# czi-ai/scldm

Hardware: AMD Instinct MI355X
Metric: cells/sec (whole node) @100 Euler steps; DiT-fwd MFMA util % of peak (higher is better)
Workload: dtype bf16; 1 GPU; dentate_b4096_euler100; cells_per_gpu=4096, global_cells=4096, cfg_evaluations=100, method=euler, sample_forwards_per_evaluation_per_gpu=12288, gathered_rows=8192, parallelism=single GPU

## Files before the change

scldm_amd/csrc/api.hip:

```cpp
#include <hip/hip_runtime.h>

#include <algorithm>
#include <cstdarg>
#include <cstdio>
#include <cstdlib>
#include <cstring>
#include <vector>

#include <cmath>
#include "api_common.hpp"
#include "dit_aux.hpp"
#include "dit_forward.hpp"
#include "dit_handle.hpp"
#include "ode_rk.hpp"

using namespace scldm;

static thread_local char g_err[512] = "";
int scldm_fail(int code, const char* fmt, ...) {
  va_list ap;
  va_start(ap, fmt);
  vsnprintf(g_err, sizeof(g_err), fmt, ap);
  va_end(ap);
  return code;
// ... 28 lines not shown
    if (cfg->n_embed % 256 != 0 || cfg->n_embed > 2048 || cfg->seq_len != 16 || (hd != 32 && hd != 64))
      return fail(SCLDM_ERR_SHAPE, "unsupported DiT shape: fused kernels need n_embed=256, n_head=8, seq_len=16; the generic path needs "
                  "n_embed %% 256 == 0 (<= 2048), seq_len=16, head_dim 32 or 64 (got n_embed=%d, n_head=%d, seq_len=%d)", cfg->n_embed,
                  cfg->n_head, cfg->seq_len);
  }
  if (cfg->n_layer < 1 || cfg->hidden_dim < 1) return fail(SCLDM_ERR_SHAPE, "bad n_layer / hidden_dim");
  if (cfg->n_classes < 0 || cfg->n_classes > SCLDM_MAX_CLASSES) return fail(SCLDM_ERR_SHAPE, "n_classes must be <= %d", SCLDM_MAX_CLASSES);
  if (cfg->has_null_row != 0 && cfg->has_null_row != 1) return fail(SCLDM_ERR_SHAPE, "has_null_row must be 0 or 1");
  for (int c = 0; c < cfg->n_classes; ++c)
    if (cfg->class_vocab[c] < 1) return fail(SCLDM_ERR_SHAPE, "class %d has an empty vocabulary", c);
  scldm_dit* h = new scldm_dit();
  h->cfg = *cfg;
  h->fused = fused;
  h->mod_w = cfg->n_layer * 6 * cfg->n_embed + 2 * cfg->n_embed;
  for (int c = 0; c < cfg->n_classes; ++c) h->tab_rows[c] = cfg->class_vocab[c] + cfg->has_null_row;
  h->bf16_sources = true;
  if (const char* e = getenv("SCLDM_TRAIN_BF16_SOURCES")) h->bf16_sources = atoi(e) != 0;
  h->wgrad_batch = true;
  if (const char* e = getenv("SCLDM_WGRAD_BATCH")) h->wgrad_batch = atoi(e) != 0;
  if (!fused) {
    *out = h;
    return SCLDM_OK;
  }
  if (const char* e = getenv("SCLDM_FT")) h->force_ft = atoi(e);
  if (const char* e = getenv("SCLDM_X3_FT")) h->force_x3_ft = atoi(e);
  if (const char* e = getenv("SCLDM_X3_NTT")) h->force_x3_ntt = atoi(e);
  if (const char* e = getenv("SCLDM_SMALL_NTT")) h->small_ntt = atoi(e) != 0;
  h->lpl = kMaxLayersPerLaunch;
  if (const char* e = getenv("SCLDM_LPL")) h->lpl = std::min(kMaxLayersPerLaunch, std::max(1, atoi(e)));
  h->groups = 1;
  if (const char* e = getenv("SCLDM_ADALN_VALU")) h->adaln_valu = atoi(e) != 0;
  if (const char* e = getenv("SCLDM_ADALN_EXACT")) h->adaln_exact = atoi(e) != 0;
  if (const char* e = getenv("SCLDM_ADALN_ROWTILE")) h->adaln_rowtile = atoi(e) != 0;
  if (const char* e = getenv("SCLDM_COND_AHEAD")) h->cond_ahead = atoi(e) != 0;
  if (const char* e = getenv("SCLDM_COND_ALL")) h->cond_all_on = atoi(e) != 0;
  if (const char* e = getenv("SCLDM_GROUPS")) h->groups = std::min(4, std::max(1, atoi(e)));
  if (const char* e = getenv("SCLDM_TAIL_SPLIT")) h->tail_split = atoi(e) != 0;
  {
    int dev = 0;
    hipDeviceProp_t prop;
    if (hipGetDevice(&dev) == hipSuccess && hipGetDeviceProperties(&prop, dev) == hipSuccess && prop.multiProcessorCount > 0)
      h->n_cu = prop.multiProcessorCount;
  }
  h->dbg_layer = -1;
  if (const char* e = getenv("SCLDM_DBG_LAYER")) h->dbg_layer = atoi(e);
  h->train_fused = true;
// ... 162 lines not shown
    j.d = dst;
    i = 0;
    for (int v : par) j.p[i++] = v;
    j.d_off = d_off;
    const int nb = cdiv(pack_job_threads(kind, n, j.p), 256);
    blocks += nb;
    jobs.push_back(j);
    if (train) {
      j.first_block = tblocks;
      tblocks += nb;
      tjobs.push_back(j);
    }
  };
  auto src = [&](const float* p, long long n) { fps.push_back(FpSrc{(const uint32_t*)p, n}); return p; };
  for (int i = 0; i < L; ++i) {
    src(w->attn_w[i], 768 * 256); src(w->proj_w[i], 256 * 256); src(w->w1[i], (long long)H * 256); src(w->w2[i], (long long)H * 256);
    src(w->cproj[i], (long long)H * 256);
    for (int p = 0; p < kNPrec; ++p)
      for (int f = 0; f < 2; ++f) {
        if (!h->stream[p][f]) continue;
        const int nc = h->n_chunks[f], hf = h->half[f];
        const long long npk = (long long)4 * units_per_layer(nc, hf) * 1024;
        train = (p == SCLDM_PREC_BF16 || p == SCLDM_PREC_FP16) && f == 1;
        add(kPackLayer, npk, {w->attn_w[i], w->proj_w[i], w->w1[i], w->w2[i], w->cproj[i]}, h->stream[p][f], {H, nc, hf, f + 1, p}, npk * i);
        train = false;
      }
    if (h->bwd_stream) {
      const long long npk = (long long)8 * kBwdUnitsLayer * 512;
      train = true;
      add(kPackLayerBwd, npk, {w->attn_w[i], w->proj_w[i], w->w1[i], w->w2[i], w->cproj[i]}, h->bwd_stream, {H}, npk * i);
    }
    train = true;
    add(kPackCopy, 768, {src(w->attn_b[i], 768)}, h->b_qkv + (size_t)i * 768, {});
    add(kPackCopy, 256, {src(w->proj_b[i], 256)}, h->b_proj + (size_t)i * 256, {});
    add(kPackTranspose, 1536 * 256, {src(w->ada_w[i], 1536 * 256)}, h->ada_t, {1536, 256, mw, i * 1536});
    add(kPackCopy, 1536, {src(w->ada_b[i], 1536)}, h->ada_b + i * 1536, {});
    train = false;
    add(kPackAdaX3, 1536 * 256, {w->ada_w[i]}, h->ada_x3, {i * 1536});
  }
  train = true;
  add(kPackTranspose, 512 * 256, {src(w->fin_ada_w, 512 * 256)}, h->ada_t, {512, 256, mw, L * 1536});
  add(kPackCopy, 512, {src(w->fin_ada_b, 512)}, h->ada_b + L * 1536, {});
  train = false;
  add(kPackAdaX3, 512 * 256, {w->fin_ada_w}, h->ada_x3, {L * 1536});
  add(kPackTranspose, 256 * 256, {src(w->t_w0, 256 * 256)}, h->w0t, {256, 256, 256, 0});
  add(kPackTranspose, 256 * 256, {src(w->t_w2, 256 * 256)}, h->w2t, {256, 256, 256, 0});
  add(kPackCopy, 256, {src(w->t_b0, 256)}, h->b0, {});
// ... 179 lines not shown
    const int n_tiles = h->mod_w / 32;
    if (rows <= 128 || !asplit || h->adaln_rowtile) {
      if (rows <= 128) adaln_x3_kernel<1><<<dim3(cdiv(n_tiles, 4), cdiv(rows, 32)), 256, 0, st>>>(silu_c, wf, h->ada_b, mod, rows, h->mod_w, rows_dev);
      else adaln_x3_kernel<4><<<dim3(cdiv(n_tiles, 16), cdiv(rows, 32)), 256, 0, st>>>(silu_c, wf, h->ada_b, mod, rows, h->mod_w, rows_dev);
    } else {
      bf16x8x2* af = reinterpret_cast<bf16x8x2*>(asplit);
      adaln_split_rows_kernel<<<cdiv(rows, 32) * 4, 256, 0, st>>>(silu_c, af, rows, rows_dev);
      adaln_x3_block_kernel<<<dim3(cdiv(n_tiles, 4), cdiv(rows, 128)), 256, 0, st>>>(af, wf, h->ada_b, mod, rows, h->mod_w, rows_dev);
    }
    LAUNCH_CHECK();
    return SCLDM_OK;
  }
  if (h->adaln_valu) {
    dim3 grid(cdiv(h->mod_w, 64), cdiv(rows, kAdaRU));
    adaln_all_kernel<<<grid, 256, 0, st>>>(silu_c, h->ada_t, h->ada_b, mod, rows, h->mod_w, rows_dev);
  } else {
    dim3 grid(cdiv(h->mod_w, 128), cdiv(rows, 32));
    adaln_mfma_kernel<<<grid, 256, 0, st>>>(silu_c, h->ada_t, h->ada_b, mod, rows, h->mod_w, rows_dev);
  }
  LAUNCH_CHECK();
  return SCLDM_OK;
}

template <typename OP, int NTT, int FT>
static int launch_fwd_t(const FwdArgs& a, hipStream_t st) {
  using L = FwdLayout<OP, NTT, FT>;
  static bool attr_set[64] = {};
  int dev = 0;
  HIP_TRY(hipGetDevice(&dev));
  if (dev < 0 || dev >= 64 || !attr_set[dev]) {
    HIP_TRY(hipFuncSetAttribute((const void*)dit_forward_kernel<OP, NTT, FT>, hipFuncAttributeMaxDynamicSharedMemorySize, L::LDS_BYTES));
    if (dev >= 0 && dev < 64) attr_set[dev] = true;
  }
  const int tiles = cdiv((long long)a.n_fwd * 16, L::TM);
  const int grid = a.grid_tiles > 0 ? a.grid_tiles : tiles;
  dit_forward_kernel<OP, NTT, FT><<<grid, L::NT, L::LDS_BYTES, st>>>(a);
  LAUNCH_CHECK();
  return SCLDM_OK;
}

static int launch_fwd(int prec, int ntt, int ft, const FwdArgs& a, hipStream_t st) {
  if (prec == SCLDM_PREC_FP32) return launch_fwd_t<OpF32, 2, 2>(a, st);
  if (prec == SCLDM_PREC_BF16X3)
    return ft == 1 ? launch_fwd_t<OpBF16x3, 2, 1>(a, st) : ntt == 1 ? launch_fwd_t<OpBF16x3, 1, 2>(a, st) : launch_fwd_t<OpBF16x3, 2, 2>(a, st);
  if (prec == SCLDM_PREC_FP16) return ft == 1 ? launch_fwd_t<OpFP16, 2, 1>(a, st) : ntt == 1 ? launch_fwd_t<OpFP16, 1, 2>(a, st) : launch_fwd_t<OpFP16, 2, 2>(a, st);
  if (ft == 1) return launch_fwd_t<OpBF16, 2, 1>(a, st);
  return ntt == 1 ? launch_fwd_t<OpBF16, 1, 2>(a, st) : launch_fwd_t<OpBF16, 2, 2>(a, st);
}

static int trunk(scldm_dit* h, const float* x, int n_direct, int rep, int n_fwd, const float* mod, const int32_t* ridx,
                 float* hbuf, float* out, int prec, hipStream_t st) {
  const scldm_dit_config& c = h->cfg;
  const size_t es = esize(prec);
  int ntt, ft;
  pick_shape(h, prec, &ntt, &ft);
  if (h->small_ntt && (prec == SCLDM_PREC_BF16 || prec == SCLDM_PREC_FP16) && ntt == 2 && ft == 2 && (long long)n_fwd * 16 <= 256 * 32) ntt = 1;
  const size_t layer_elems = (size_t)4 * units_per_layer(h->n_chunks[ft - 1], h->half[ft - 1]) * 1024;
  FwdArgs a{};
  a.z = x;
  a.out = out;
  a.x = hbuf;
  a.mod = mod;
  a.row_index = ridx;
  a.w_final = h->wfinal[prec];
  a.in_wt = h->in_wt;
  a.in_w = h->in_w;
  a.in_b = h->in_b;
  a.pos = h->pos;
  a.fin_b = h->fin_b;
// ... 49 lines not shown
    a.w_stream = (const char*)h->stream[prec][ft - 1] + (size_t)i * layer_elems * es;
    a.b_qkv = h->b_qkv + (size_t)i * 768;
    a.b_proj = h->b_proj + (size_t)i * 256;
    hipEvent_t e0 = nullptr, e1 = nullptr;
    if (h->timing && h->ev_used + 2 <= 40000) {
      while (h->ev.size() < h->ev_used + 2) {
        hipEvent_t ev;
        HIP_TRY(hipEventCreate(&ev));
        h->ev.push_back(ev);
      }
      e0 = h->ev[h->ev_used];
      e1 = h->ev[h->ev_used + 1];
      h->ev_used += 2;
      HIP_TRY(hipEventRecord(e0, st));
    }
    int rc = SCLDM_OK;
    if (tail_full > 0) {
      hipStream_t s1 = st;
      if (n64 > 0) {
        HIP_TRY(hipEventRecord(h->fork_ev, st));
        HIP_TRY(hipStreamWaitEvent(h->side[0], h->fork_ev, 0));
        a.tile0 = 0;
        a.grid_tiles = n64;
        rc = launch_fwd(prec, 2, ft, a, st);
        s1 = h->side[0];
      }
      a.tile0 = 2 * n64;
      a.grid_tiles = n32;
      if (rc == SCLDM_OK) rc = launch_fwd(prec, 1, ft, a, s1);
      if (n64 > 0) {
        HIP_TRY(hipEventRecord(h->join_ev[0], h->side[0]));
        HIP_TRY(hipStreamWaitEvent(st, h->join_ev[0], 0));
      }
      a.tile0 = 0;
      a.grid_tiles = 0;
    } else
      for (int g = 0; g < G && rc == SCLDM_OK; ++g) {
        hipStream_t sg = g == 0 ? st : h->side[g - 1];
        if (G > 1) {
          a.tile0 = gt0[g];
          a.grid_tiles = gt0[g + 1] - gt0[g];
        }
        rc = launch_fwd(prec, ntt, ft, a, sg);
      }
    if (rc != SCLDM_OK) return rc;
    if (e1) HIP_TRY(hipEventRecord(e1, st));
  }
  if (G > 1)
    for (int g = 1; g < G; ++g) {
      HIP_TRY(hipEventRecord(h->join_ev[g - 1], h->side[g - 1]));
      HIP_TRY(hipStreamWaitEvent(st, h->join_ev[g - 1], 0));
    }
  return SCLDM_OK;
}

static int check_ready(const scldm_dit* h, int prec) {
  if (!h) return fail(SCLDM_ERR_SHAPE, "null handle");
  if (!h->loaded) return fail(SCLDM_ERR_STATE, "scldm_dit_load_weights has not been called");
  if (prec != SCLDM_PREC_FP32 && prec != SCLDM_PREC_BF16 && prec != SCLDM_PREC_BF16X3 && prec != SCLDM_PREC_FP16) return fail(SCLDM_ERR_SHAPE, "unknown precision %d", prec);
  if (!h->fused) return fail(SCLDM_ERR_SHAPE, "this handle's shape is outside the fused family (scldm_dit_train_* only)");
  return SCLDM_OK;
}

extern "C" int scldm_dit_cond_rows(scldm_dit* h, const float* t, int t_stride, const int64_t* const* labels, int n_rows,
                                   float* mod_out, void* ws_, void* stream_) {
  int rc = check_ready(h, 0);
// ... 473 lines not shown
```

scldm_amd/csrc/common.hpp:

```cpp
#pragma once
#include <hip/hip_runtime.h>
#include <stdint.h>

namespace scldm {

typedef __attribute__((ext_vector_type(16))) float f32x16;
typedef __attribute__((ext_vector_type(8))) float f32x8;
typedef __attribute__((ext_vector_type(4))) float f32x4;
typedef __attribute__((ext_vector_type(8))) __bf16 bf16x8;
typedef __attribute__((ext_vector_type(4))) __bf16 bf16x4;

constexpr int kWave = 64;

__device__ __forceinline__ int acc_row(int r, int hh) { return (r & 3) + 8 * (r >> 2) + 4 * hh; }

__device__ __forceinline__ float silu_f(float x) { return x * __builtin_amdgcn_rcpf(1.0f + __builtin_amdgcn_exp2f(-1.4426950408889634f * x)); }

__device__ __forceinline__ float xor32_sum(float v) {
  const auto r = __builtin_amdgcn_permlane32_swap(__float_as_uint(v), __float_as_uint(v), false, false);
  return __uint_as_float(r[0]) + __uint_as_float(r[1]);
}
__device__ __forceinline__ float xor32_max(float v) {
  const auto r = __builtin_amdgcn_permlane32_swap(__float_as_uint(v), __float_as_uint(v), false, false);
  return fmaxf(__uint_as_float(r[0]), __uint_as_float(r[1]));
// ... 23 lines not shown
struct OpBF16 {
  using E = __bf16;
  using ModE = _Float16;
  static __device__ __forceinline__ f32x4 load_mod4(const ModE* p) {
    const f16x4 h = *reinterpret_cast<const f16x4*>(p);
    return f32x4{(float)h[0], (float)h[1], (float)h[2], (float)h[3]};
  }
  static __device__ __forceinline__ void store_mod4(ModE* p, const f32x4 v) {
    *reinterpret_cast<f16x4*>(p) = f16x4{(_Float16)v[0], (_Float16)v[1], (_Float16)v[2], (_Float16)v[3]};
  }
  using Frag = bf16x8;
  using Quad = bf16x4;
  static constexpr bool kIsBF16 = true;
  static constexpr bool kTwoPassLN = false;
  static constexpr bool kPin = true;
  static constexpr bool kMfmaIn = true;
  static constexpr bool kTwoWG = true;
  static constexpr int kRing = 4;
  static constexpr int kFragLoads = 1;
  static constexpr int kMmaOps = 1;
  static __device__ __forceinline__ f32x16 mma(const Frag& a, const Frag& b, f32x16 c) {
    return __builtin_amdgcn_mfma_f32_32x32x16_bf16(a, b, c, 0, 0, 0);
  }
  static constexpr float kW1Scale = -1.4426950408889634f, kW2Scale = -0.6931471805599453f;
  static __device__ __forceinline__ float swiglu(float a, float b) { return (a * b) * __builtin_amdgcn_rcpf(1.0f + __builtin_amdgcn_exp2f(a)); }
  static __device__ __forceinline__ void store_quad(E* row, int f, const Quad& q) { *reinterpret_cast<Quad*>(row + f) = q; }
  static __device__ __forceinline__ void store_quad_pair(E* row, int f8, int hh, const Quad& q0, const Quad& q1) {
    union { Quad q; unsigned u[2]; } a, b;
    a.q = q0; b.q = q1;
    halfwave_pair(a.u[0], b.u[0]);
    halfwave_pair(a.u[1], b.u[1]);
    typedef __attribute__((ext_vector_type(4))) unsigned u32x4;
    *reinterpret_cast<u32x4*>(row + f8 + 8 * hh) = u32x4{a.u[0], a.u[1], b.u[0], b.u[1]};
  }
  static __device__ __forceinline__ Frag pack8(const float* v) {
    Frag f;
#pragma unroll
    for (int i = 0; i < 8; ++i) f[i] = (__bf16)v[i];
    return f;
  }
  static __device__ __forceinline__ Quad pack4(float a, float b, float c, float d) {
    Quad q;
    q[0] = (__bf16)a; q[1] = (__bf16)b; q[2] = (__bf16)c; q[3] = (__bf16)d;
    return q;
  }
};

struct OpFP16 {
  using E = _Float16;
  using ModE = _Float16;
  static __device__ __forceinline__ f32x4 load_mod4(const ModE* p) {
    const f16x4 h = *reinterpret_cast<const f16x4*>(p);
    return f32x4{(float)h[0], (float)h[1], (float)h[2], (float)h[3]};
  }
  static __device__ __forceinline__ void store_mod4(ModE* p, const f32x4 v) {
    *reinterpret_cast<f16x4*>(p) = f16x4{(_Float16)v[0], (_Float16)v[1], (_Float16)v[2], (_Float16)v[3]};
  }
  using Frag = f16x8;
  using Quad = f16x4;
  static constexpr bool kIsBF16 = true;
  static constexpr bool kTwoPassLN = false;
  static constexpr bool kPin = true;
  static constexpr bool kMfmaIn = true;
  static constexpr bool kTwoWG = true;
  static constexpr int kRing = 4;
  static constexpr int kFragLoads = 1;
  static constexpr int kMmaOps = 1;
  static __device__ __forceinline__ f32x16 mma(const Frag& a, const Frag& b, f32x16 c) {
    return __builtin_amdgcn_mfma_f32_32x32x16_f16(a, b, c, 0, 0, 0);
  }
  static constexpr float kW1Scale = -1.4426950408889634f, kW2Scale = -0.6931471805599453f;
  static __device__ __forceinline__ float swiglu(float a, float b) { return (a * b) * __builtin_amdgcn_rcpf(1.0f + __builtin_amdgcn_exp2f(a)); }
  static __device__ __forceinline__ void store_quad(E* row, int f, const Quad& q) { *reinterpret_cast<Quad*>(row + f) = q; }
  static __device__ __forceinline__ void store_quad_pair(E* row, int f8, int hh, const Quad& q0, const Quad& q1) {
    union { Quad q; unsigned u[2]; } a, b;
    a.q = q0; b.q = q1;
    halfwave_pair(a.u[0], b.u[0]);
    halfwave_pair(a.u[1], b.u[1]);
    typedef __attribute__((ext_vector_type(4))) unsigned u32x4;
    *reinterpret_cast<u32x4*>(row + f8 + 8 * hh) = u32x4{a.u[0], a.u[1], b.u[0], b.u[1]};
  }
  static __device__ __forceinline__ Frag pack8(const float* v) {
    Frag f;
#pragma unroll
    for (int i = 0; i < 8; ++i) f[i] = (_Float16)v[i];
    return f;
  }
  static __device__ __forceinline__ Quad pack4(float a, float b, float c, float d) {
    Quad q;
    q[0] = (_Float16)a; q[1] = (_Float16)b; q[2] = (_Float16)c; q[3] = (_Float16)d;
    return q;
  }
// ... 113 lines not shown
```

scldm_amd/csrc/dit_aux.hpp:

```cpp
#pragma once
#include "common.hpp"
#include "dit_forward.hpp"
#include "bwd_layout.hpp"

namespace scldm {

__device__ __forceinline__ float pack_layer_val(const float* __restrict__ Wqkv, const float* __restrict__ Wproj,
                                                const float* __restrict__ W1, const float* __restrict__ W2,
                                                const float* __restrict__ Wcp, long long idx, int H, int n_chunks, int half, int FT,
                                                float s1, float s2) {
  const int UL = units_per_layer(n_chunks, half), unit_elems = 512 * FT;
  const int j = idx & 7, l = (idx >> 3) & 63, ft = (int)((idx >> 9) % FT);
  const int gu = (int)(idx / unit_elems), w = gu / UL, u = gu % UL;
  const int r = l & 31, k8 = (l >> 5) * 8 + j;
  const int frow = (w * FT + ft) * 32 + r;
  float val;
  if (u < 32 && FT == 2) {
    const int head = u >> 4, ks = u & 15;
    val = Wqkv[(size_t)(ft * 256 + (w * 2 + head) * 32 + r) * 256 + ks * 16 + k8];
  } else if (u < 48) {
    const int p = u >> 4, ks = u & 15;
    val = Wqkv[(size_t)(p * 256 + frow) * 256 + ks * 16 + k8];
  } else if (u < 64) {
    const int ks = u - 48;
    val = Wproj[(size_t)frow * 256 + ks * 16 + k8];
  } else if (u >= 64 + n_chunks * kUnitsPerChunk) {
    const int vh = u - 64 - n_chunks * kUnitsPerChunk, hid0 = n_chunks * kHC;
    if (vh < 8) {
      const int ks = 2 * vh + ft, hid = hid0 + w * 16 + (r & 15);
      const float* src = (r < 16) ? W1 : W2;
      val = (hid < H) ? src[(size_t)hid * 256 + ks * 16 + k8] * ((r < 16) ? s1 : s2) : 0.f;
    } else {
      const int hid = hid0 + (vh - 8) * 16 + k8;
      val = (hid < H) ? Wcp[(size_t)frow * H + hid] : 0.f;
    }
  } else {
    const int v = u - 64, c = v / kUnitsPerChunk, vv = v % kUnitsPerChunk;
    if (vv < 16) {
      const int tile = (FT == 2 && !SCLDM_W12_PAIR) ? (vv >> 3) : ft;
      const int ks = (FT == 2 && !SCLDM_W12_PAIR) ? (2 * (vv & 7) + ft) : vv;
      const int hid = c * kHC + (w * FT + tile) * 16 + (r & 15);
      const float* src = (r < 16) ? W1 : W2;
      val = (hid < H) ? src[(size_t)hid * 256 + ks * 16 + k8] * ((r < 16) ? s1 : s2) : 0.f;
    } else {
      const int hid = c * kHC + (vv - 16) * 16 + k8;
      val = (hid < H) ? Wcp[(size_t)frow * H + hid] : 0.f;
    }
  }
  return val;
}

__device__ __forceinline__ float pack_bwd_val(const float* __restrict__ Wqkv, const float* __restrict__ Wproj,
                                              const float* __restrict__ W1, const float* __restrict__ W2,
                                              const float* __restrict__ Wcp, long long idx, int H) {
  const int j = idx & 7, l = (idx >> 3) & 63;
  const int gu = (int)(idx >> 9), w = gu / kBwdUnitsLayer, u = gu % kBwdUnitsLayer;
  const int r = l & 31, k8 = (l >> 5) * 8 + j;
  const int frow = w * 32 + r;
  if (u < kBwdChunks * kBwdUnitsChunk) {
    const int c = u / kBwdUnitsChunk, v = u % kBwdUnitsChunk;
    const int hid = c * kBwdChunk + w * 32 + r;
// ... 134 lines not shown
      const int n = (int)(idx >> 8) + j.p[0], k = (int)(idx & 255);
      const float v = j.s[0][idx];
      __bf16 hi, lo;
      OpBF16x3::split(v, hi, lo);
      const size_t base = ((((size_t)(n >> 5) * 16 + (k >> 4)) * 64 + ((k >> 3) & 1) * 32 + (n & 31)) << 4) + (k & 7);
      reinterpret_cast<__bf16*>(j.d)[base] = hi;
      reinterpret_cast<__bf16*>(j.d)[base + 8] = lo;
      break;
    }
    case kPackLayerBwd: {
      if (!(prec_mask & 0x100u)) return;
      float v[8];
#pragma unroll
      for (int e = 0; e < 8; ++e) v[e] = pack_bwd_val(j.s[0], j.s[1], j.s[2], j.s[3], j.s[4], idx * 8 + e, j.p[0]);
      pack_store8(j.d, j.d_off / 8 + idx, v, (prec_mask & 0x200u) ? 3 : 1);
      break;
    }
    case kPackLayer:
      if (!((prec_mask >> j.p[4]) & 1u)) return;
      {
        const float s1 = (j.p[4] == 1 || j.p[4] == 3) ? OpBF16::kW1Scale : 1.0f, s2 = (j.p[4] == 1 || j.p[4] == 3) ? OpBF16::kW2Scale : 1.0f;
        float v[8];
#pragma unroll
        for (int e = 0; e < 8; ++e) v[e] = pack_layer_val(j.s[0], j.s[1], j.s[2], j.s[3], j.s[4], idx * 8 + e, j.p[0], j.p[1], j.p[2], j.p[3], s1, s2);
        pack_store8(j.d, j.d_off / 8 + idx, v, j.p[4], fp16_stats);
      }
      break;
    case kPackFinal: {
      if (!((prec_mask >> j.p[1]) & 1u)) return;
      const int jj = idx & 7, l = (idx >> 3) & 63, ks = (int)(idx >> 9);
      const int row = l & 31, k = ks * 16 + (l >> 5) * 8 + jj;
      pack_store(j.d, idx, (row < j.p[0]) ? j.s[0][row * 256 + k] : 0.f, j.p[1], fp16_stats);
      break;
    }
  }
}

constexpr int kFpSplit = 32;
struct FpSrc {
  const uint32_t* p;
  long long n;
};
__global__ __launch_bounds__(256) void fingerprint_kernel(const FpSrc* __restrict__ src, unsigned long long* __restrict__ acc) {
  const FpSrc s = src[blockIdx.x];
  if (s.n <= 0) return;
  long long chunk = ((s.n + kFpSplit - 1) / kFpSplit + 255) / 256 * 256;
  if (chunk < 2048) chunk = 2048;
// ... 430 lines not shown
```

scldm_amd/csrc/dit_forward.hpp:

```cpp
#pragma once
#include <type_traits>

#include "common.hpp"

#ifndef SCLDM_SETPRIO
#define SCLDM_SETPRIO 1
#endif
#ifndef SCLDM_BPF
#define SCLDM_BPF 1
#endif
#ifndef SCLDM_LEAN_VALU
#define SCLDM_LEAN_VALU 1
#endif
#ifndef SCLDM_PAIR_STORE
#define SCLDM_PAIR_STORE 1
#endif

#pragma clang fp contract(off)

namespace scldm {

constexpr int kD = 256;
constexpr int kHC = 128;
constexpr int kModBlock = 6 * kD;
// ... 266 lines not shown
      }
      if (OP::kPin) {
        __builtin_amdgcn_sched_group_barrier(0x100, NTT * OP::kFragLoads, 0);
        __builtin_amdgcn_sched_group_barrier(0x008, NTT * OP::kMmaOps, 0);
        if (half == 1) __builtin_amdgcn_sched_group_barrier(0x020, 2 * OP::kFragLoads, 0);
      }
    }
  };
#if SCLDM_SETPRIO
  __builtin_amdgcn_s_setprio(SCLDM_SETPRIO);
#endif
#pragma unroll
  for (int s = 0; s < PF; ++s) unit(s, s, s == 0);
#pragma unroll 1
  for (int u0 = PF; u0 < UNITS; u0 += PF) {
#pragma unroll
    for (int s = 0; s < PF; ++s) unit(u0 + s, s, false);
  }
#if SCLDM_SETPRIO
  __builtin_amdgcn_s_setprio(0);
#endif
}

#ifdef SCLDM_PHASE_TIMING
#define SCLDM_LN_STAMP(i)                                                                              \
  do {                                                                                                 \
    if (SB >= 0 && dbg && lane == 0) dbg[((size_t)blockIdx.x * 8 + wave) * kDbgStamps + SB + (i)] = __builtin_readcyclecounter(); \
  } while (0)
#else
#define SCLDM_LN_STAMP(i) do {} while (0)
#endif

template <typename OP, int NTT, int FT, int SB = -1, typename Between>
__device__ __forceinline__ void ln_modulate_store(const float (&v)[FT][NTT][16], const typename OP::ModE* msm, int sc_v, int sh_v,
                                                  float eps, float* red, typename OP::E* dst, int ldd, int wave,
                                                  int lane, unsigned long long* dbg, Between between) {
  constexpr int TM = 32 * NTT;
  constexpr int NW = 8 / FT;
  const int c32 = lane & 31, hh = lane >> 5;
  float* red_a = red;
  float* red_b = red + NW * TM;
  float mean[NTT], rstd[NTT];
  if (OP::kTwoPassLN) {
#pragma unroll
    for (int tt = 0; tt < NTT; ++tt) {
      float s = 0.f;
// ... 98 lines not shown
#pragma unroll
      for (int i = 0; i < 4; ++i) y[i] = fmaf(fmaf(v[ft][tt][q * 4 + i], rstd[tt], nmr[tt]), sc[i], sh[i]);
    } else {
#pragma unroll
      for (int i = 0; i < 4; ++i) y[i] = fmaf((v[ft][tt][q * 4 + i] - mean[tt]) * rstd[tt], sc[i], sh[i]);
    }
#else
#pragma unroll
    for (int i = 0; i < 4; ++i) y[i] = (v[ft][tt][q * 4 + i] - mean[tt]) * rstd[tt] * (1.0f + sc[i]) + sh[i];
#endif
#if SCLDM_PAIR_STORE
    const typename OP::Quad packed = OP::pack4(y[0], y[1], y[2], y[3]);
    if ((q & 1) == 0) held = packed;
    else OP::store_quad_pair(dst + (tt * 32 + c32) * ldd, (wave * FT + ft) * 32 + (q - 1) * 8, hh, held, packed);
#else
    OP::store_quad(dst + (tt * 32 + c32) * ldd, f, OP::pack4(y[0], y[1], y[2], y[3]));
#endif
  }
}

#ifndef SCLDM_FWD_ONE_WG
#define SCLDM_FWD_ONE_WG 0
#endif
template <typename OP, int NTT, int FT, bool REC = false>
__global__ __launch_bounds__(64 * (8 / FT), (!SCLDM_FWD_ONE_WG && ((OP::kTwoWG && NTT <= 2) || NTT == 1)) ? 2 : 1) void dit_forward_kernel(const FwdArgs a) {
  using L = FwdLayout<OP, NTT, FT>;
  using E = typename OP::E;
  using Frag = typename OP::Frag;
  using Quad = typename OP::Quad;
  constexpr int TM = L::TM;
  constexpr int NS = L::NS;
  constexpr int NW = L::NW;
  constexpr int NT = L::NT;
  constexpr int PF = Prefetch<OP, NTT, FT>::PF;

  extern __shared__ __attribute__((aligned(16))) char smem[];
  E* XA = reinterpret_cast<E*>(smem);
  E* HB = reinterpret_cast<E*>(smem + L::XA_BYTES);
  using ModE = typename OP::ModE;
  float* RED = reinterpret_cast<float*>(smem + L::RED_OFF);
  ModE* MOD = reinterpret_cast<ModE*>(smem + L::MOD_OFF);
  E* AO = XA;

  const int tid = threadIdx.x;
  const int lane = tid & 63;
  const int wave = __builtin_amdgcn_readfirstlane(tid >> 6);
  const int tile_id = blockIdx.x + a.tile0;
  const int tok0 = tile_id * TM;
// ... 424 lines not shown
  SCLDM_STAMP(8);

  f32x16 accp[FT][NTT];
  auto do_chunk = [&](auto half_tag, int c) {
    constexpr bool HALF = decltype(half_tag)::value;
    constexpr int TILES = (FT == 2 && HALF) ? 1 : FT;
    Quad hq[TILES][NTT][2];
    constexpr bool kPair = SCLDM_W12_PAIR != 0;
    auto swiglu_pack = [&](const f32x16 (&t_acc)[NTT], Quad (&out)[NTT][2]) {
#pragma unroll
      for (int tt = 0; tt < NTT; ++tt)
#pragma unroll
        for (int q = 0; q < 2; ++q) {
          float h[4];
#pragma unroll
#if SCLDM_PROXY & 4
          for (int i = 0; i < 4; ++i) h[i] = t_acc[tt][q * 4 + i] * t_acc[tt][8 + q * 4 + i];
#else
          for (int i = 0; i < 4; ++i) h[i] = OP::swiglu(t_acc[tt][q * 4 + i], t_acc[tt][8 + q * 4 + i]);
#endif
          out[tt][q] = OP::pack4(h[0], h[1], h[2], h[3]);
        }
    };
    if constexpr (FT == 2) {
      if constexpr (HALF || !kPair) {
#pragma unroll
        for (int ft = 0; ft < TILES; ++ft) {
          f32x16 a1[NTT];
          gemm_pass_tile<OP, NTT, PF>(a1, ws, XA, L::XA_LD, lane);
          swiglu_pack(a1, hq[ft]);
        }
      } else {
        gemm_pass<OP, NTT, FT, 16, false, true, PF>(acc, ws, XA, L::XA_LD, lane);
#pragma unroll
        for (int ft = 0; ft < TILES; ++ft) swiglu_pack(acc[ft], hq[ft]);
      }
    } else {
      gemm_pass<OP, NTT, FT, 16, false, true, PF>(acc, ws, XA, L::XA_LD, lane);
#pragma unroll
      for (int ft = 0; ft < FT; ++ft) swiglu_pack(acc[ft], hq[ft]);
    }
    E* HBc = HB + (L::HB_BUFS == 2 ? (c & 1) * (L::HB_BYTES / (int)sizeof(E)) : 0);
    if (L::HB_BUFS == 1 && c > 0) lds_barrier();
#pragma unroll
    for (int ft = 0; ft < TILES; ++ft) {
      const int col0 = HALF ? wave * 16 : (wave * FT + ft) * 16;
#pragma unroll
      for (int tt = 0; tt < NTT; ++tt) {
#if SCLDM_PAIR_STORE
        OP::store_quad_pair(HBc + (tt * 32 + c32) * L::HB_LD, col0, hh, hq[ft][tt][0], hq[ft][tt][1]);
#else
#pragma unroll
        for (int q = 0; q < 2; ++q)
          OP::store_quad(HBc + (tt * 32 + c32) * L::HB_LD, col0 + q * 8 + hh * 4, hq[ft][tt][q]);
#endif
      }
    }
    if (c == 0) SCLDM_STAMP(11);
    lds_barrier();
    if (c == 0) SCLDM_STAMP(12);
    constexpr int KS = HALF ? 4 : 8;
    if (c == 0) gemm_pass<OP, NTT, FT, KS, false, true, PF>(accp, ws, HBc, L::HB_LD, lane);
    else gemm_pass<OP, NTT, FT, KS, false, false, PF>(accp, ws, HBc, L::HB_LD, lane);
    if (c == 0) SCLDM_STAMP(13);
  };
  for (int c = 0; c < a.n_chunks; ++c) do_chunk(std::false_type{}, c);
  if (a.half_chunk) do_chunk(std::true_type{}, a.n_chunks);
  SCLDM_STAMP(9);

// ... 88 lines not shown
```

scldm_amd/csrc/dit_handle.hpp:

```cpp
#pragma once
#include <hip/hip_runtime.h>

#include <vector>

#include "../../include/scldm_hip.h"

struct scldm_dit {
  scldm_dit_config cfg;
  int n_chunks[2], half[2];
  int mod_w;
  bool loaded;
  bool fused;
  void* stream[4][2];
  void* wfinal[4];
  float *b_qkv, *b_proj;
  float *w0t, *b0, *w2t, *b2;
  float* emb;
  int emb_row0[SCLDM_MAX_CLASSES];
  float *ada_t, *ada_b;
  void* ada_x3;
  float *in_wt, *in_b, *pos;
  float* in_w;
  float* fin_b;
  bool timing;
  std::vector<hipEvent_t> ev;
  size_t ev_used;
  int lpl;
  bool adaln_rowtile = false;
  bool adaln_exact = false;
  bool adaln_valu = false;
  int cfg1_direct = 0;
  int tail_split = 0;
  int n_cu = 256;
  int groups;
  int dbg_layer;
  int tab_rows[SCLDM_MAX_CLASSES];
// ... 57 lines not shown
```

scldm_amd/csrc/train_fused.hip:

```cpp
#include "train_fused.hpp"

#include <hip/hip_runtime.h>

#include <algorithm>
#include <cstdio>
#include <cstdlib>
#include <vector>

#include "api_common.hpp"
#define SCLDM_BWD_NS bwd
#define SCLDM_BWD_OP OpBF16
#include "dit_backward.hpp"
#undef SCLDM_BWD_NS
#undef SCLDM_BWD_OP
#define SCLDM_BWD_NS bwdh
#define SCLDM_BWD_OP OpFP16
#include "dit_backward.hpp"
#undef SCLDM_BWD_NS
#undef SCLDM_BWD_OP
#define SCLDM_BWD_NTT 1
#define SCLDM_BWD_NS bwd32
#define SCLDM_BWD_OP OpBF16
#include "dit_backward.hpp"
#undef SCLDM_BWD_NS
// ... 598 lines not shown
int join_side(scldm_dit* h, hipStream_t st, int k) {
  HIP_TRY(hipEventRecord(h->join_ev[k], h->side[k]));
  HIP_TRY(hipStreamWaitEvent(st, h->join_ev[k], 0));
  return SCLDM_OK;
}
int prepare_join(scldm_dit* h, hipStream_t st) {
  HIP_TRY(hipStreamWaitEvent(st, h->join_ev[0], 0));
  return SCLDM_OK;
}
int backward_join(scldm_dit* h, hipStream_t st) {
  if (h->bwd_pack_ev) HIP_TRY(hipStreamWaitEvent(st, h->bwd_pack_ev, 0));
  return SCLDM_OK;
}

int forward(scldm_dit* h, const float* x, const float* mod, int n, float* out, const Record& rec, const Scratch& s, hipStream_t st, int precision) {
  using L = FwdLayout<OpBF16, 2, 2>;
  using L1 = FwdLayout<OpBF16, 1, 2>;
  static_assert(FwdLayout<OpFP16, 2, 2>::LDS_BYTES == L::LDS_BYTES && FwdLayout<OpFP16, 2, 2>::NT == L::NT, "fp16 = the bf16 kernel's shape");
  static_assert(FwdLayout<OpFP16, 1, 2>::LDS_BYTES == L1::LDS_BYTES && L1::NT == L::NT, "fp16 = the bf16 kernel's shape");
  const bool f16 = precision == SCLDM_PREC_FP16;
  static const bool small_ok = [] { const char* e = getenv("SCLDM_TRAIN_SMALL_NTT"); return !(e && e[0] == '0'); }();
  const int tiles64 = pad4(n) / 4;
  const bool small = small_ok && tiles64 <= 128;
  void (*kern)(const FwdArgs) = small ? (f16 ? dit_forward_kernel<OpFP16, 1, 2, true> : dit_forward_kernel<OpBF16, 1, 2, true>)
                                      : (f16 ? dit_forward_kernel<OpFP16, 2, 2, true> : dit_forward_kernel<OpBF16, 2, 2, true>);
  const int lds_bytes = small ? L1::LDS_BYTES : L::LDS_BYTES;
  static bool attr_set[2][2][64] = {};
  int dev = 0;
  HIP_TRY(hipGetDevice(&dev));
  if (dev < 0 || dev >= 64 || !attr_set[small][f16][dev]) {
    HIP_TRY(hipFuncSetAttribute((const void*)kern, hipFuncAttributeMaxDynamicSharedMemorySize, lds_bytes));
    if (dev >= 0 && dev < 64) attr_set[small][f16][dev] = true;
  }
  const scldm_dit_config& c = h->cfg;
  if (h->iota_n < n) {
    HIP_TRY(hipStreamSynchronize(st));
    if (h->iota) (void)hipFree(h->iota);
    h->iota = nullptr;
    h->iota_n = 0;
    const int cap = std::max(n, 4096);
    HIP_TRY(hipMalloc((void**)&h->iota, (size_t)cap * sizeof(int32_t)));
    iota32_kernel<<<cdiv(cap, 256), 256, 0, st>>>(h->iota, cap);
    LAUNCH_CHECK();
    h->iota_n = cap;
  }
  const size_t layer_elems = (size_t)4 * units_per_layer(h->n_chunks[1], h->half[1]) * 1024;
  FwdArgs a{};
  a.z = x;
  a.out = out;
  a.x = s.handoff;
  a.mod = mod;
  a.row_index = h->iota;
  a.w_final = h->wfinal[precision];
  a.in_wt = h->in_wt;
  a.in_w = h->in_w;
// ... 327 lines not shown
```

Baseline: 17170 cells/s.

## Use 16x16x32 MFMA for the SwiGLU up-projection with matching weight packing

Adds a forward up-projection path (W1/W2 SwiGLU GEMM) that uses 16x16x32 bf16/fp16 MFMA instructions instead of 32x32x16, with a new gemm_pass_tile16 routine and a matching weight-pack layout for FT=2 streams. It is on by default (fwd_m16=true) and can be turned off with SCLDM_FWD_MFMA=32. The smaller MFMA tile changes how the accumulators map to rows and columns, which may cut register pressure or improve issue efficiency. In exchange it needs more B-fragment LDS reads per FLOP and a separate packed weight layout.

```diff
diff --git a/scldm_amd/csrc/api.hip b/scldm_amd/csrc/api.hip
--- a/scldm_amd/csrc/api.hip
+++ b/scldm_amd/csrc/api.hip
@@ -74,6 +74,7 @@
     *out = h;
     return SCLDM_OK;
   }
+  if (const char* e = getenv("SCLDM_FWD_MFMA")) h->fwd_m16 = atoi(e) != 32;
   if (const char* e = getenv("SCLDM_FT")) h->force_ft = atoi(e);
   if (const char* e = getenv("SCLDM_X3_FT")) h->force_x3_ft = atoi(e);
   if (const char* e = getenv("SCLDM_X3_NTT")) h->force_x3_ntt = atoi(e);
@@ -282,7 +283,8 @@
         const int nc = h->n_chunks[f], hf = h->half[f];
         const long long npk = (long long)4 * units_per_layer(nc, hf) * 1024;
         train = (p == SCLDM_PREC_BF16 || p == SCLDM_PREC_FP16) && f == 1;
-        add(kPackLayer, npk, {w->attn_w[i], w->proj_w[i], w->w1[i], w->w2[i], w->cproj[i]}, h->stream[p][f], {H, nc, hf, f + 1, p}, npk * i);
+        const int m16 = h->fwd_m16 && f == 1 && (p == SCLDM_PREC_BF16 || p == SCLDM_PREC_FP16);
+        add(kPackLayer, npk, {w->attn_w[i], w->proj_w[i], w->w1[i], w->w2[i], w->cproj[i]}, h->stream[p][f], {H, nc, hf, f + 1, p, m16}, npk * i);
         train = false;
       }
     if (h->bwd_stream) {
@@ -508,29 +510,34 @@
   return SCLDM_OK;
 }
 
-template <typename OP, int NTT, int FT>
+template <typename OP, int NTT, int FT, bool M16 = false>
 static int launch_fwd_t(const FwdArgs& a, hipStream_t st) {
   using L = FwdLayout<OP, NTT, FT>;
   static bool attr_set[64] = {};
   int dev = 0;
   HIP_TRY(hipGetDevice(&dev));
   if (dev < 0 || dev >= 64 || !attr_set[dev]) {
-    HIP_TRY(hipFuncSetAttribute((const void*)dit_forward_kernel<OP, NTT, FT>, hipFuncAttributeMaxDynamicSharedMemorySize, L::LDS_BYTES));
+    HIP_TRY(hipFuncSetAttribute((const void*)dit_forward_kernel<OP, NTT, FT, false, M16>, hipFuncAttributeMaxDynamicSharedMemorySize, L::LDS_BYTES));
     if (dev >= 0 && dev < 64) attr_set[dev] = true;
   }
   const int tiles = cdiv((long long)a.n_fwd * 16, L::TM);
   const int grid = a.grid_tiles > 0 ? a.grid_tiles : tiles;
-  dit_forward_kernel<OP, NTT, FT><<<grid, L::NT, L::LDS_BYTES, st>>>(a);
+  dit_forward_kernel<OP, NTT, FT, false, M16><<<grid, L::NT, L::LDS_BYTES, st>>>(a);
   LAUNCH_CHECK();
   return SCLDM_OK;
 }
 
-static int launch_fwd(int prec, int ntt, int ft, const FwdArgs& a, hipStream_t st) {
+static int launch_fwd(int prec, int ntt, int ft, bool m16, const FwdArgs& a, hipStream_t st) {
   if (prec == SCLDM_PREC_FP32) return launch_fwd_t<OpF32, 2, 2>(a, st);
   if (prec == SCLDM_PREC_BF16X3)
     return ft == 1 ? launch_fwd_t<OpBF16x3, 2, 1>(a, st) : ntt == 1 ? launch_fwd_t<OpBF16x3, 1, 2>(a, st) : launch_fwd_t<OpBF16x3, 2, 2>(a, st);
-  if (prec == SCLDM_PREC_FP16) return ft == 1 ? launch_fwd_t<OpFP16, 2, 1>(a, st) : ntt == 1 ? launch_fwd_t<OpFP16, 1, 2>(a, st) : launch_fwd_t<OpFP16, 2, 2>(a, st);
+  if (prec == SCLDM_PREC_FP16) {
+    if (ft == 1) return launch_fwd_t<OpFP16, 2, 1>(a, st);
+    if (m16) return ntt == 1 ? launch_fwd_t<OpFP16, 1, 2, true>(a, st) : launch_fwd_t<OpFP16, 2, 2, true>(a, st);
+    return ntt == 1 ? launch_fwd_t<OpFP16, 1, 2>(a, st) : launch_fwd_t<OpFP16, 2, 2>(a, st);
+  }
   if (ft == 1) return launch_fwd_t<OpBF16, 2, 1>(a, st);
+  if (m16) return ntt == 1 ? launch_fwd_t<OpBF16, 1, 2, true>(a, st) : launch_fwd_t<OpBF16, 2, 2, true>(a, st);
   return ntt == 1 ? launch_fwd_t<OpBF16, 1, 2>(a, st) : launch_fwd_t<OpBF16, 2, 2>(a, st);
 }
 
@@ -626,12 +633,12 @@
         HIP_TRY(hipStreamWaitEvent(h->side[0], h->fork_ev, 0));
         a.tile0 = 0;
         a.grid_tiles = n64;
-        rc = launch_fwd(prec, 2, ft, a, st);
+        rc = launch_fwd(prec, 2, ft, h->fwd_m16, a, st);
         s1 = h->side[0];
       }
       a.tile0 = 2 * n64;
       a.grid_tiles = n32;
-      if (rc == SCLDM_OK) rc = launch_fwd(prec, 1, ft, a, s1);
+      if (rc == SCLDM_OK) rc = launch_fwd(prec, 1, ft, h->fwd_m16, a, s1);
       if (n64 > 0) {
         HIP_TRY(hipEventRecord(h->join_ev[0], h->side[0]));
         HIP_TRY(hipStreamWaitEvent(st, h->join_ev[0], 0));
@@ -645,7 +652,7 @@
           a.tile0 = gt0[g];
           a.grid_tiles = gt0[g + 1] - gt0[g];
         }
-        rc = launch_fwd(prec, ntt, ft, a, sg);
+        rc = launch_fwd(prec, ntt, ft, h->fwd_m16, a, sg);
       }
     if (rc != SCLDM_OK) return rc;
     if (e1) HIP_TRY(hipEventRecord(e1, st));
diff --git a/scldm_amd/csrc/common.hpp b/scldm_amd/csrc/common.hpp
--- a/scldm_amd/csrc/common.hpp
+++ b/scldm_amd/csrc/common.hpp
@@ -69,6 +69,9 @@
   static __device__ __forceinline__ f32x16 mma(const Frag& a, const Frag& b, f32x16 c) {
     return __builtin_amdgcn_mfma_f32_32x32x16_bf16(a, b, c, 0, 0, 0);
   }
+  static __device__ __forceinline__ f32x4 mma16(const Frag& a, const Frag& b, f32x4 c) {
+    return __builtin_amdgcn_mfma_f32_16x16x32_bf16(a, b, c, 0, 0, 0);
+  }
   static constexpr float kW1Scale = -1.4426950408889634f, kW2Scale = -0.6931471805599453f;
   static __device__ __forceinline__ float swiglu(float a, float b) { return (a * b) * __builtin_amdgcn_rcpf(1.0f + __builtin_amdgcn_exp2f(a)); }
   static __device__ __forceinline__ void store_quad(E* row, int f, const Quad& q) { *reinterpret_cast<Quad*>(row + f) = q; }
@@ -115,6 +118,9 @@
   static constexpr int kMmaOps = 1;
   static __device__ __forceinline__ f32x16 mma(const Frag& a, const Frag& b, f32x16 c) {
     return __builtin_amdgcn_mfma_f32_32x32x16_f16(a, b, c, 0, 0, 0);
+  }
+  static __device__ __forceinline__ f32x4 mma16(const Frag& a, const Frag& b, f32x4 c) {
+    return __builtin_amdgcn_mfma_f32_16x16x32_f16(a, b, c, 0, 0, 0);
   }
   static constexpr float kW1Scale = -1.4426950408889634f, kW2Scale = -0.6931471805599453f;
   static __device__ __forceinline__ float swiglu(float a, float b) { return (a * b) * __builtin_amdgcn_rcpf(1.0f + __builtin_amdgcn_exp2f(a)); }
diff --git a/scldm_amd/csrc/dit_aux.hpp b/scldm_amd/csrc/dit_aux.hpp
--- a/scldm_amd/csrc/dit_aux.hpp
+++ b/scldm_amd/csrc/dit_aux.hpp
@@ -8,7 +8,7 @@
 __device__ __forceinline__ float pack_layer_val(const float* __restrict__ Wqkv, const float* __restrict__ Wproj,
                                                 const float* __restrict__ W1, const float* __restrict__ W2,
                                                 const float* __restrict__ Wcp, long long idx, int H, int n_chunks, int half, int FT,
-                                                float s1, float s2) {
+                                                float s1, float s2, bool m16 = false) {
   const int UL = units_per_layer(n_chunks, half), unit_elems = 512 * FT;
   const int j = idx & 7, l = (idx >> 3) & 63, ft = (int)((idx >> 9) % FT);
   const int gu = (int)(idx / unit_elems), w = gu / UL, u = gu % UL;
@@ -26,7 +26,10 @@
     val = Wproj[(size_t)frow * 256 + ks * 16 + k8];
   } else if (u >= 64 + n_chunks * kUnitsPerChunk) {
     const int vh = u - 64 - n_chunks * kUnitsPerChunk, hid0 = n_chunks * kHC;
-    if (vh < 8) {
+    if (vh < 8 && m16) {
+      const int hid = hid0 + w * 16 + (l & 15);
+      val = (hid < H) ? (ft == 0 ? W1 : W2)[(size_t)hid * 256 + vh * 32 + (l >> 4) * 8 + j] * (ft == 0 ? s1 : s2) : 0.f;
+    } else if (vh < 8) {
       const int ks = 2 * vh + ft, hid = hid0 + w * 16 + (r & 15);
       const float* src = (r < 16) ? W1 : W2;
       val = (hid < H) ? src[(size_t)hid * 256 + ks * 16 + k8] * ((r < 16) ? s1 : s2) : 0.f;
@@ -36,7 +39,10 @@
     }
   } else {
     const int v = u - 64, c = v / kUnitsPerChunk, vv = v % kUnitsPerChunk;
-    if (vv < 16) {
+    if (vv < 16 && m16) {
+      const int hid = c * kHC + (w * 2 + (vv >> 3)) * 16 + (l & 15);
+      val = (hid < H) ? (ft == 0 ? W1 : W2)[(size_t)hid * 256 + (vv & 7) * 32 + (l >> 4) * 8 + j] * (ft == 0 ? s1 : s2) : 0.f;
+    } else if (vv < 16) {
       const int tile = (FT == 2 && !SCLDM_W12_PAIR) ? (vv >> 3) : ft;
       const int ks = (FT == 2 && !SCLDM_W12_PAIR) ? (2 * (vv & 7) + ft) : vv;
       const int hid = c * kHC + (w * FT + tile) * 16 + (r & 15);
@@ -217,7 +223,8 @@
         const float s1 = (j.p[4] == 1 || j.p[4] == 3) ? OpBF16::kW1Scale : 1.0f, s2 = (j.p[4] == 1 || j.p[4] == 3) ? OpBF16::kW2Scale : 1.0f;
         float v[8];
 #pragma unroll
-        for (int e = 0; e < 8; ++e) v[e] = pack_layer_val(j.s[0], j.s[1], j.s[2], j.s[3], j.s[4], idx * 8 + e, j.p[0], j.p[1], j.p[2], j.p[3], s1, s2);
+        for (int e = 0; e < 8; ++e) v[e] = pack_layer_val(j.s[0], j.s[1], j.s[2], j.s[3], j.s[4], idx * 8 + e, j.p[0], j.p[1], j.p[2], j.p[3], s1, s2,
+                                                        j.p[3] == 2 && j.p[5] != 0);
         pack_store8(j.d, j.d_off / 8 + idx, v, j.p[4], fp16_stats);
       }
       break;
diff --git a/scldm_amd/csrc/dit_forward.hpp b/scldm_amd/csrc/dit_forward.hpp
--- a/scldm_amd/csrc/dit_forward.hpp
+++ b/scldm_amd/csrc/dit_forward.hpp
@@ -312,6 +312,53 @@
 #endif
 }
 
+template <typename OP, int NTT, int PF>
+__device__ __forceinline__ void gemm_pass_tile16(f32x4 (&a1)[2 * NTT], f32x4 (&b1)[2 * NTT], WStream<OP, PF, 2>& ws,
+                                                 const typename OP::E* __restrict__ bsm, int ldb, int lane) {
+  using Frag = typename OP::Frag;
+  constexpr int UNITS = 8, NJ = 2 * NTT;
+  static_assert(UNITS % PF == 0, "8 units must be a multiple of the prefetch depth");
+  const typename OP::E* bbase = bsm + (lane & 15) * ldb + (lane >> 4) * 8;
+  const f32x4 zero = {0.f, 0.f, 0.f, 0.f};
+  Frag bcur[NJ];
+#pragma unroll
+  for (int j = 0; j < NJ; ++j) bcur[j] = *reinterpret_cast<const Frag*>(bbase + j * 16 * ldb);
+  auto unit = [&](int u, int s, bool first) {
+#pragma unroll
+    for (int j = 0; j < NJ; ++j) {
+      a1[j] = OP::mma16(ws.ring[s][0], bcur[j], first ? zero : a1[j]);
+      b1[j] = OP::mma16(ws.ring[s][1], bcur[j], first ? zero : b1[j]);
+      bcur[j] = *reinterpret_cast<const Frag*>(bbase + j * 16 * ldb + ((u + 1) & (UNITS - 1)) * 32);
+    }
+#if !(SCLDM_PROXY & 1)
+    ws.ring[s][0] = ws.fetch(0);
+    ws.ring[s][1] = ws.fetch(1);
+#endif
+    ws.advance(2);
+    if (OP::kPin) {
+#pragma unroll
+      for (int j = 0; j < NJ; ++j) {
+        __builtin_amdgcn_sched_group_barrier(0x008, 2, 0);
+        __builtin_amdgcn_sched_group_barrier(0x100, OP::kFragLoads, 0);
+      }
+      __builtin_amdgcn_sched_group_barrier(0x020, 2 * OP::kFragLoads, 0);
+    }
+  };
+#if SCLDM_SETPRIO
+  __builtin_amdgcn_s_setprio(SCLDM_SETPRIO);
+#endif
+#pragma unroll
+  for (int s = 0; s < PF; ++s) unit(s, s, s == 0);
+#pragma unroll 1
+  for (int u0 = PF; u0 < UNITS; u0 += PF) {
+#pragma unroll
+    for (int s = 0; s < PF; ++s) unit(u0 + s, s, false);
+  }
+#if SCLDM_SETPRIO
+  __builtin_amdgcn_s_setprio(0);
+#endif
+}
+
 #ifdef SCLDM_PHASE_TIMING
 #define SCLDM_LN_STAMP(i)                                                                              \
   do {                                                                                                 \
@@ -456,8 +503,9 @@
 #ifndef SCLDM_FWD_ONE_WG
 #define SCLDM_FWD_ONE_WG 0
 #endif
-template <typename OP, int NTT, int FT, bool REC = false>
+template <typename OP, int NTT, int FT, bool REC = false, bool M16 = false>
 __global__ __launch_bounds__(64 * (8 / FT), (!SCLDM_FWD_ONE_WG && ((OP::kTwoWG && NTT <= 2) || NTT == 1)) ? 2 : 1) void dit_forward_kernel(const FwdArgs a) {
+  static_assert(!M16 || (FT == 2 && sizeof(typename OP::E) == 2 && sizeof(typename OP::Frag) == 16), "M16: 16-bit policies, FT = 2");
   using L = FwdLayout<OP, NTT, FT>;
   using E = typename OP::E;
   using Frag = typename OP::Frag;
@@ -928,7 +976,19 @@
           out[tt][q] = OP::pack4(h[0], h[1], h[2], h[3]);
         }
     };
-    if constexpr (FT == 2) {
+    Quad hq16[M16 ? TILES : 1][M16 ? 2 * NTT : 1];
+    if constexpr (M16) {
+      static_assert(HALF || !kPair, "M16: one-tile up-projection passes");
+#pragma unroll
+      for (int ft = 0; ft < TILES; ++ft) {
+        f32x4 a1[2 * NTT], b1[2 * NTT];
+        gemm_pass_tile16<OP, NTT, PF>(a1, b1, ws, XA, L::XA_LD, lane);
+#pragma unroll
+        for (int j = 0; j < 2 * NTT; ++j)
+          hq16[ft][j] = OP::pack4(OP::swiglu(a1[j][0], b1[j][0]), OP::swiglu(a1[j][1], b1[j][1]), OP::swiglu(a1[j][2], b1[j][2]),
+                                  OP::swiglu(a1[j][3], b1[j][3]));
+      }
+    } else if constexpr (FT == 2) {
       if constexpr (HALF || !kPair) {
 #pragma unroll
         for (int ft = 0; ft < TILES; ++ft) {
@@ -951,6 +1011,11 @@
 #pragma unroll
     for (int ft = 0; ft < TILES; ++ft) {
       const int col0 = HALF ? wave * 16 : (wave * FT + ft) * 16;
+      if constexpr (M16) {
+#pragma unroll
+        for (int j = 0; j < 2 * NTT; ++j) OP::store_quad(HBc + (j * 16 + (lane & 15)) * L::HB_LD, col0 + (lane >> 4) * 4, hq16[ft][j]);
+        continue;
+      }
 #pragma unroll
       for (int tt = 0; tt < NTT; ++tt) {
 #if SCLDM_PAIR_STORE
diff --git a/scldm_amd/csrc/dit_handle.hpp b/scldm_amd/csrc/dit_handle.hpp
--- a/scldm_amd/csrc/dit_handle.hpp
+++ b/scldm_amd/csrc/dit_handle.hpp
@@ -12,6 +12,7 @@
   bool loaded;
   bool fused;
   void* stream[4][2];
+  bool fwd_m16 = true;
   void* wfinal[4];
   float *b_qkv, *b_proj;
   float *w0t, *b0, *w2t, *b2;
diff --git a/scldm_amd/csrc/train_fused.hip b/scldm_amd/csrc/train_fused.hip
--- a/scldm_amd/csrc/train_fused.hip
+++ b/scldm_amd/csrc/train_fused.hip
@@ -644,15 +644,19 @@
   static const bool small_ok = [] { const char* e = getenv("SCLDM_TRAIN_SMALL_NTT"); return !(e && e[0] == '0'); }();
   const int tiles64 = pad4(n) / 4;
   const bool small = small_ok && tiles64 <= 128;
-  void (*kern)(const FwdArgs) = small ? (f16 ? dit_forward_kernel<OpFP16, 1, 2, true> : dit_forward_kernel<OpBF16, 1, 2, true>)
-                                      : (f16 ? dit_forward_kernel<OpFP16, 2, 2, true> : dit_forward_kernel<OpBF16, 2, 2, true>);
+  const bool m16 = h->fwd_m16;
+  void (*kern)(const FwdArgs) =
+      m16 ? (small ? (f16 ? dit_forward_kernel<OpFP16, 1, 2, true, true> : dit_forward_kernel<OpBF16, 1, 2, true, true>)
+                   : (f16 ? dit_forward_kernel<OpFP16, 2, 2, true, true> : dit_forward_kernel<OpBF16, 2, 2, true, true>))
+          : (small ? (f16 ? dit_forward_kernel<OpFP16, 1, 2, true> : dit_forward_kernel<OpBF16, 1, 2, true>)
+                   : (f16 ? dit_forward_kernel<OpFP16, 2, 2, true> : dit_forward_kernel<OpBF16, 2, 2, true>));
   const int lds_bytes = small ? L1::LDS_BYTES : L::LDS_BYTES;
-  static bool attr_set[2][2][64] = {};
+  static bool attr_set[2][2][2][64] = {};
   int dev = 0;
   HIP_TRY(hipGetDevice(&dev));
-  if (dev < 0 || dev >= 64 || !attr_set[small][f16][dev]) {
+  if (dev < 0 || dev >= 64 || !attr_set[m16][small][f16][dev]) {
     HIP_TRY(hipFuncSetAttribute((const void*)kern, hipFuncAttributeMaxDynamicSharedMemorySize, lds_bytes));
-    if (dev >= 0 && dev < 64) attr_set[small][f16][dev] = true;
+    if (dev >= 0 && dev < 64) attr_set[m16][small][f16][dev] = true;
   }
   const scldm_dit_config& c = h->cfg;
   if (h->iota_n < n) {
```

New measurement: 17710 cells/s, median of 6. +3.1%, better.
